# coganlab/cross_patient_speech_decoding

Hardware: AMD Instinct MI355X
Metric: ECoG trials/sec seq2seq-RNN training (higher is better)
Workload: dtype bf16x3; 1 GPU; configs[3] per-GPU shard: 8-patient MCCA-aligned input (d = 30), enc 2x bi-GRU H=512, dec 1x GRU, T=200 (T'=20), F=100, full-batch step of 2048 trials per GPU (8 patients x 2048 trials over 8 GPUs), dropout 0.3, teacher forcing 0.5, clip 0.5, AdamW; trials_per_gpu=2048, global_batch=2048, parallelism=dp1, collective=none (single process)

## Files before the change

### cross_patient_speech_decoding_amd/csrc/xps_gemm.hip

```cpp
#include <stdlib.h>
#include <string.h>
#include <atomic>
#include "xps_common.h"
#include "xps_gemm_tile.h"
#include "xps_gemm_big.h"
#include "xps_gemm_dma.h"
using namespace xps_tile;
#ifndef XPS_GEMM_DEFAULT_MODE
#define XPS_GEMM_DEFAULT_MODE 1
#endif
namespace {

#ifndef XPS_BF_MI1_WAVES
#define XPS_BF_MI1_WAVES XPS_GEMM_WAVES
#endif
template <bool AK, bool BK, int MI, bool EDGE = false, bool BF = false, bool PRE = false>
__global__ __launch_bounds__(256, (BF && MI == 1) ? XPS_BF_MI1_WAVES : XPS_GEMM_WAVES) void gemm_f32_kernel(
    const float* __restrict__ A, RowMap ra, const float* __restrict__ B, RowMap rb,
    const float* __restrict__ A2, const float* __restrict__ B2, int K2,
    float* __restrict__ C, RowMap rc, const float* __restrict__ bias,
    int M, int N, int K, int kchunk, long long slab_stride, int accumulate, int vecA, int vecB) {
    __shared__ __attribute__((aligned(16))) TileMem<BF, MI> mem;
    const int tiles_n = (N + BN - 1) / BN, tiles = tiles_n * ((M + 64 * MI - 1) / (64 * MI));
    const int lid = xcd_remap(blockIdx.x, gridDim.x);
    const int z = lid / tiles, t = lid % tiles;
    const int kbeg = z * kchunk;
    const int kend = min(K, kbeg + kchunk);
    const int m0 = (t / tiles_n) * (64 * MI), n0 = (t % tiles_n) * BN;
    f32x16 acc[MI][2];
    zero_acc<MI>(acc);
    float nocs = 0.f;
    f32x4 nocs4 = {0.f, 0.f, 0.f, 0.f};
    gemm_accumulate_any<AK, BK, MI, EDGE, BF, PRE>(acc, nocs, nocs4, false, A, ra, B, rb, M, N, K, m0, n0, kbeg, kend, vecA, vecB, mem);
    if (A2) gemm_accumulate_any<AK, BK, MI, EDGE, BF, PRE>(acc, nocs, nocs4, false, A2, ra, B2, rb, M, N, K2, m0, n0, 0, K2, vecA, vecB, mem);
    gemm_store<MI>(acc, C + (long long)z * slab_stride, rc, bias, M, N, m0, n0, accumulate);
}

constexpr int SM_MAXM = 16, SM_SLICES = 16, SM_KC = 1024;
template <bool AK, bool BK>
__global__ __launch_bounds__(1024) void gemm_small_kernel(
    const float* __restrict__ A, RowMap ra, const float* __restrict__ B, RowMap rb,
    const float* __restrict__ A2, const float* __restrict__ B2, int K2,
    float* __restrict__ C, RowMap rc, const float* __restrict__ bias, int M, int N, int K, int accumulate, int vecB) {
    __shared__ __attribute__((aligned(16))) float As[SM_MAXM][SM_KC];
    __shared__ float red[SM_SLICES][SM_MAXM][64];
    const int tid = threadIdx.x, l = tid & 63, w = tid >> 6;
    const int n = blockIdx.x * 64 + l;
    float acc[SM_MAXM];
#pragma unroll
    for (int m = 0; m < SM_MAXM; ++m) acc[m] = 0.f;
    for (int pass = 0; pass < 2; ++pass) {
        const float* __restrict__ Ap = pass ? A2 : A;
// ... 27 lines not shown
                    }
#pragma unroll
                    for (int m = 0; m < SM_MAXM; ++m) {
                        const f32x4 a = *reinterpret_cast<const f32x4*>(&As[m][k]);
                        acc[m] += a.x * b[0]; acc[m] += a.y * b[1]; acc[m] += a.z * b[2]; acc[m] += a.w * b[3];
                    }
                }
                for (; k < k1; ++k) {
                    const float b = BK ? Bp[boff + k] : Bp[(plain_b ? (long long)(kc + k) * rb.ld : rb.off(kc + k)) + boff];
#pragma unroll
                    for (int m = 0; m < SM_MAXM; ++m) acc[m] += As[m][k] * b;
                }
            }
        }
    }
#pragma unroll
    for (int m = 0; m < SM_MAXM; ++m) red[w][m][l] = acc[m];
    __syncthreads();
    if (w < M && n < N) {
        float v = 0.f;
#pragma unroll
        for (int s = 0; s < SM_SLICES; ++s) v += red[s][w][l];
        if (bias) v += bias[n];
        float* c = C + rc.off(w) + n;
        if (accumulate) v += *c;
        *c = v;
    }
}

struct NtMulti {
    const float* B[4];
    const float* bias[4];
    float* C[4];
};
template <int MI, bool EDGE = false, bool BF = false, bool PRE = false>
__global__ __launch_bounds__(256, (BF && MI == 1) ? XPS_BF_MI1_WAVES : XPS_GEMM_WAVES) void gemm_nt_multi_kernel(
    const float* __restrict__ A, RowMap ra, NtMulti pm, RowMap rb, RowMap rc, int M, int N, int K, int nprob,
    int vecA, int vecB) {
    __shared__ __attribute__((aligned(16))) TileMem<BF, MI> mem;
    const int tiles_n = (N + BN - 1) / BN;
    const int lid = xcd_remap(blockIdx.x, gridDim.x);
    const int per_m = nprob * tiles_n, rem = lid % per_m;
    const int z = rem / tiles_n;
    const int m0 = (lid / per_m) * (64 * MI), n0 = (rem % tiles_n) * BN;
    f32x16 acc[MI][2];
    zero_acc<MI>(acc);
    float nocs = 0.f;
    f32x4 nocs4 = {0.f, 0.f, 0.f, 0.f};
    gemm_accumulate_any<true, true, MI, EDGE, BF, PRE>(acc, nocs, nocs4, false, A, ra, pm.B[z], rb, M, N, K, m0, n0, 0, K, vecA, vecB, mem);
    gemm_store<MI>(acc, pm.C[z], rc, pm.bias[z], M, N, m0, n0, 0);
}


template <int KT>
__global__ __launch_bounds__(512, 1) void proj_ws_kernel(const float* __restrict__ A, long long lda, NtMulti pm, long long ldb, long long ldc,
                                                         int M, int N, int K, int nprob, int preA, int preB) {
    constexpr int KP = 16 * KT;
#ifndef XPS_WS_PAD
#define XPS_WS_PAD 4
#endif
    constexpr int LDH = ((KP / 2 + 63) / 64) * 64 + XPS_WS_PAD;
    constexpr int NV = KP / 32;
    extern __shared__ __attribute__((aligned(16))) unsigned char ws_smem[];
    unsigned* lds = reinterpret_cast<unsigned*>(ws_smem);
    const int tid = threadIdx.x, lane = tid & 63, wave = tid >> 6;
    const int NC = nprob * N, S = (NC + 255) / 256;
    const int lid = xcd_remap(blockIdx.x, gridDim.x);
    const int slice = lid % S, rg = lid / S;
    const int nb = (gridDim.x - slice + S - 1) / S;
    const int c0 = slice * 256 + wave * 32;
    const bool active = c0 < NC;
    const int z = active ? c0 / N : 0, n0 = active ? c0 % N : 0;
    const int li = lane & 31, lk = lane >> 5;

    bf16x8 wh[KT], wl[KT];
    {
        const float* wrow = pm.B[z] + (long long)(n0 + li) * ldb;
#pragma unroll
        for (int kk = 0; kk < KT; ++kk) {
            const int k = 16 * kk + 8 * lk;
            f32x4 v0 = {0.f, 0.f, 0.f, 0.f}, v1 = v0;
            if (active && k < K) v0 = *reinterpret_cast<const f32x4*>(wrow + k);
            if (active && k + 4 < K) v1 = *reinterpret_cast<const f32x4*>(wrow + k + 4);
            bf16x4 h0, l0, h1, l1;
            stage_split(v0, preB != 0, h0, l0);
            stage_split(v1, preB != 0, h1, l1);
            wh[kk] = __builtin_shufflevector(h0, h1, 0, 1, 2, 3, 4, 5, 6, 7);
            wl[kk] = __builtin_shufflevector(l0, l1, 0, 1, 2, 3, 4, 5, 6, 7);
        }
    }
    float bv = 0.f;
    if (active && pm.bias[z]) bv = pm.bias[z][n0 + li];

    const int tiles = (M + 63) / 64;
    auto load_tile = [&](int t, f32x4 (&r)[NV]) {
#pragma unroll
        for (int j = 0; j < NV; ++j) {
            const int v = tid + 512 * j, row = t * 64 + v / (KP / 4), k = 4 * (v % (KP / 4));
            r[j] = (row < M && k < K) ? *reinterpret_cast<const f32x4*>(A + (long long)row * lda + k) : f32x4{0.f, 0.f, 0.f, 0.f};
        }
    };
    auto store_tile = [&](const f32x4 (&r)[NV], int buf) {
        unsigned* hi = lds + (size_t)buf * 2 * 64 * LDH;
        unsigned* lo = hi + 64 * LDH;
#pragma unroll
        for (int j = 0; j < NV; ++j) {
            const int v = tid + 512 * j, row = v / (KP / 4), kd = 2 * (v % (KP / 4));
            bf16x4 h, l;
            stage_split(r[j], preA != 0, h, l);
            *reinterpret_cast<bf16x4*>(hi + row * LDH + kd) = h;
            *reinterpret_cast<bf16x4*>(lo + row * LDH + kd) = l;
        }
    };

    f32x4 raw[NV];
    int t = rg;
    if (t < tiles) load_tile(t, raw);
    for (int it = 0; t < tiles; t += nb, ++it) {
        const int buf = it & 1;
        store_tile(raw, buf);
        if (t + nb < tiles) load_tile(t + nb, raw);
        __syncthreads();
        if (active) {
            const unsigned* hi = lds + (size_t)buf * 2 * 64 * LDH;
            const unsigned* lo = hi + 64 * LDH;
            f32x16 acc[2];
#pragma unroll
            for (int i = 0; i < 2; ++i)
#pragma unroll
                for (int r = 0; r < 16; ++r) acc[i][r] = 0.f;
#pragma unroll
            for (int kk = 0; kk < KT; ++kk) {
#pragma unroll
                for (int i = 0; i < 2; ++i) {
                    const int off = (32 * i + li) * LDH + 8 * kk + 4 * lk;
                    const bf16x8 ah = *reinterpret_cast<const bf16x8*>(hi + off);
                    const bf16x8 al = *reinterpret_cast<const bf16x8*>(lo + off);
                    acc[i] = __builtin_amdgcn_mfma_f32_32x32x16_bf16(al, wh[kk], acc[i], 0, 0, 0);
                    acc[i] = __builtin_amdgcn_mfma_f32_32x32x16_bf16(ah, wl[kk], acc[i], 0, 0, 0);
                    acc[i] = __builtin_amdgcn_mfma_f32_32x32x16_bf16(ah, wh[kk], acc[i], 0, 0, 0);
                }
            }
            float* cbase = pm.C[z] + n0 + li;
#pragma unroll
            for (int i = 0; i < 2; ++i)
#pragma unroll
                for (int r = 0; r < 16; ++r) {
                    const int row = t * 64 + 32 * i + (r & 3) + 8 * (r >> 2) + 4 * lk;
                    if (row < M) __builtin_nontemporal_store(acc[i][r] + bv, cbase + (long long)row * ldc);
                }
        }
    }
}
constexpr int proj_ws_lds(int KT) { return 2 * 2 * 64 * (((16 * KT / 2 + 63) / 64) * 64 + XPS_WS_PAD) * 4; }

constexpr int TN_MAXP = 12;
struct TnProb {
    const float* A; const float* B; float* C; float* colsum;
    RowMap ra, rb, rc;
    int M, N, K, accumulate;
    int splits, kchunk, tiles_n, vecA, vecB;
    long long slab_off;
    int block_start;
    int big;
};
struct TnGroup {
    TnProb p[TN_MAXP];
    int n;
    int total_blocks;
    int total_blocks_big;
    long long total_out;
    int uniform, tiles_all;
    int tile_start[TN_MAXP];
};

constexpr int TN_TILE = BM * BN;
__host__ __device__ inline long long tn_split_stride(long long ntiles, int M, bool has_colsum) {
    return ntiles * TN_TILE + (has_colsum ? ((M + 3) & ~3) : 0);
}
__device__ inline void slab_store(const f32x16 (&acc)[2][2], float* __restrict__ tile) {
    const int lane = threadIdx.x & 63, wave = threadIdx.x >> 6;
    float* base = tile + wave * 4096 + lane * 4;
#pragma unroll
    for (int i = 0; i < 2; ++i)
#pragma unroll
        for (int j = 0; j < 2; ++j)
#pragma unroll
            for (int q = 0; q < 4; ++q) {
                const f32x4 v = {acc[i][j][4 * q], acc[i][j][4 * q + 1], acc[i][j][4 * q + 2], acc[i][j][4 * q + 3]};
                __builtin_nontemporal_store(v, reinterpret_cast<f32x4*>(base + ((i * 2 + j) * 4 + q) * 256));
            }
}
__device__ inline void slab_decode(int e, int& row, int& col) {
    const int wave = e >> 12, ij = (e >> 10) & 3, q = (e >> 8) & 3, lane = (e >> 2) & 63, c = e & 3;
    const int reg = 4 * q + c, li = lane & 31, lk = lane >> 5;
    row = (wave >> 1) * 64 + (ij >> 1) * 32 + (reg & 3) + 8 * (reg >> 2) + 4 * lk;
    col = (wave & 1) * 64 + (ij & 1) * 32 + li;
}

template <bool EDGE, bool BF = false, bool PRE = false>
__global__ __launch_bounds__(256, XPS_GEMM_WAVES) void gemm_tn_grouped_kernel(TnGroup g, float* __restrict__ ws) {
    __shared__ __attribute__((aligned(16))) TileMem<BF> mem;
    const int lid = xcd_remap(blockIdx.x, gridDim.x);
    int pi = 0, local;
    if (g.uniform) {
        const int zz = lid / g.tiles_all, rem = lid - zz * g.tiles_all;
#pragma unroll 1
// ... 179 lines not shown
    }
}

extern __shared__ __attribute__((aligned(16))) unsigned char big_smem[];

template <bool AK, bool BK, bool DEEP, int FMT = -1>
__device__ inline void big_accumulate(f32x16 (&acc)[4][2], f32x4& csum, bool want_csum, const float* __restrict__ A, long long lda,
                                      const float* __restrict__ B, long long ldb, int m0, int n0, int kbeg, int kend,
                                      const bool preA = false, const bool preB = false) {
    if constexpr (DEEP) {
        xps_big::BigStage32& st = *reinterpret_cast<xps_big::BigStage32*>(big_smem);
        xps_big::BigLoader32<AK> la;
        xps_big::BigLoader32<BK> lb;
        la.init(A, lda, m0, kbeg, threadIdx.x);
        lb.init(B, ldb, n0, kbeg, threadIdx.x);
        xps_big::big_pipeline32<AK, BK>(acc, csum, want_csum, la, lb, (kend - kbeg) / 32, st, preA, preB);
    } else {
        xps_big::BigStage& st = *reinterpret_cast<xps_big::BigStage*>(big_smem);
        xps_big::BigLoader<AK> la;
        xps_big::BigLoader<BK> lb;
        la.init(A, lda, m0, kbeg, threadIdx.x);
        lb.init(B, ldb, n0, kbeg, threadIdx.x);
        if constexpr (FMT >= 0) xps_big::big_pipeline_t<AK, BK, (FMT & 1) != 0, (FMT & 2) != 0>(acc, csum, want_csum, la, lb, (kend - kbeg) / BKT, st);
        else xps_big::big_pipeline<AK, BK>(acc, csum, want_csum, la, lb, (kend - kbeg) / BKT, st, preA, preB);
    }
}

template <bool AK, bool BK, bool DEEP, int FMT = 0>
__global__ __launch_bounds__(512, 1) void gemm_big_kernel(const float* __restrict__ A, long long lda, const float* __restrict__ B,
                                                           long long ldb, const float* __restrict__ A2, const float* __restrict__ B2,
                                                           int K2, float* __restrict__ C, long long ldc,
                                                           const float* __restrict__ bias, int N, int K, int accumulate, int fmt) {
    const int tiles_n = FMT == 5 ? 1 : N / xps_big::TN;
    const int lid = xcd_remap(blockIdx.x, gridDim.x);
    const int m0 = (lid / tiles_n) * xps_big::TM, n0 = (lid % tiles_n) * xps_big::TN;
    f32x16 acc[4][2];
    xps_big::big_zero(acc);
    f32x4 nocs = {0.f, 0.f, 0.f, 0.f};
    if constexpr (FMT == 5) {
        const bool act = (int)((threadIdx.x >> 6) & 3) * 64 < N;
        xps_big::direct_dma_pipeline<!BK>(acc, A, lda, B, ldb, m0, 0, 0, K / 32, big_smem, act);
        if (A2) xps_big::direct_dma_pipeline<!BK>(acc, A2, lda, B2, ldb, m0, 0, 0, K2 / 32, big_smem, act);
        xps_big::big_store_c_masked(acc, C, ldc, bias, m0, N, accumulate);
        return;
    }
    if constexpr (FMT == 4) {
        xps_big::direct_dma_pipeline<!BK>(acc, A, lda, B, ldb, m0, n0, 0, K / 32, big_smem);
        if (A2) xps_big::direct_dma_pipeline<!BK>(acc, A2, lda, B2, ldb, m0, n0, 0, K2 / 32, big_smem);
    } else {
        big_accumulate<AK, BK, DEEP, DEEP ? -1 : FMT>(acc, nocs, false, A, lda, B, ldb, m0, n0, 0, K, !DEEP && (fmt & 1) != 0, !DEEP && (fmt & 2) != 0);
        if (A2) big_accumulate<AK, BK, DEEP, DEEP ? -1 : FMT>(acc, nocs, false, A2, lda, B2, ldb, m0, n0, 0, K2, !DEEP && (fmt & 1) != 0, !DEEP && (fmt & 2) != 0);
    }
    xps_big::big_store_c(acc, C, ldc, bias, m0, n0, accumulate);
}

template <bool DEEP, bool DMA = false>
__global__ __launch_bounds__(512, 1) void gemm_big_nt_multi_kernel(const float* __restrict__ A, long long lda, NtMulti pm, long long ldb,
                                                                    long long ldc, int N, int K, int nprob, int fmt) {
    const int tiles_n = N / xps_big::TN;
    const int lid = xcd_remap(blockIdx.x, gridDim.x);
    const int per_m = nprob * tiles_n, rem = lid % per_m;
    const int z = rem / tiles_n;
    const int m0 = (lid / per_m) * xps_big::TM, n0 = (rem % tiles_n) * xps_big::TN;
    f32x16 acc[4][2];
    xps_big::big_zero(acc);
    f32x4 nocs = {0.f, 0.f, 0.f, 0.f};
    if constexpr (DMA) xps_big::direct_dma_pipeline<false>(acc, A, lda, pm.B[z], ldb, m0, n0, 0, K / 32, big_smem);
    else big_accumulate<true, true, DEEP>(acc, nocs, false, A, lda, pm.B[z], ldb, m0, n0, 0, K, !DEEP && (fmt & 1) != 0, !DEEP && (fmt & 2) != 0);
    xps_big::big_store_c(acc, pm.C[z], ldc, pm.bias[z], m0, n0, 0);
}

template <bool DEEP>
__global__ __launch_bounds__(512, 1) void gemm_big_tn_kernel(TnGroup g, float* __restrict__ ws) {
    const int lid = xcd_remap(blockIdx.x, gridDim.x);
    int pi = -1;
#pragma unroll 1
    for (int i = 0; i < g.n; ++i)
        if (g.p[i].big && lid >= g.p[i].block_start) pi = i;
    const TnProb& P = g.p[pi];
    const int local = lid - P.block_start;
    const int tiles_n = P.N / xps_big::TN, ntiles = (P.M / xps_big::TM) * tiles_n;
    const int tile = local % ntiles, z = local / ntiles;
    const int tm = tile / tiles_n, tn = tile % tiles_n;
    const int kbeg = z * P.kchunk, kend = min(P.K, kbeg + P.kchunk);
    const long long ntiles128 = (long long)(P.M / BM) * P.tiles_n;
    const long long split_stride = tn_split_stride(ntiles128, P.M, P.colsum != nullptr);
    float* slab = ws + P.slab_off + (long long)z * split_stride;
    const bool want_cs = P.colsum && tn == 0;
    f32x16 acc[4][2];
    xps_big::big_zero(acc);
    if (!DEEP && P.big == 2) {
        f32x16 cacc;
#pragma unroll
        for (int r = 0; r < 16; ++r) cacc[r] = 0.f;
        const int per = (8 + tiles_n - 1) / tiles_n;
        const int cs_lo = min(8, tn * per), cs_hi = min(8, cs_lo + per);
        const bool cs_here = P.colsum && cs_lo < cs_hi;
        if (cs_here) xps_big::tn_dma_pipeline<true>(acc, cacc, P.A, P.ra.ld, P.B, P.rb.ld, tm * xps_big::TM, tn * xps_big::TN, kbeg, (kend - kbeg) / BKT, big_smem, cs_lo, cs_hi);
        else xps_big::tn_dma_pipeline<false>(acc, cacc, P.A, P.ra.ld, P.B, P.rb.ld, tm * xps_big::TM, tn * xps_big::TN, kbeg, (kend - kbeg) / BKT, big_smem);
        float* subd[4];
#pragma unroll
        for (int s = 0; s < 4; ++s)
            subd[s] = slab + ((long long)(2 * tm + (s >> 1)) * P.tiles_n + 2 * tn + (s & 1)) * TN_TILE;
        xps_big::big_slab_store(acc, subd);
        if (cs_here) xps_big::dma_colsum_store(cacc, slab + ntiles128 * TN_TILE + tm * xps_big::TM, cs_lo, cs_hi);
        return;
// ... 39 lines not shown
inline bool aligned16(const void* p) { return (reinterpret_cast<uintptr_t>(p) & 15) == 0; }
inline bool map_vec_ok(const float* p, const RowMap& r) {
    return aligned16(p) && (r.ld % 4 == 0) && (r.gs % 4 == 0);
}
inline int split4_flag(const float* p, const RowMap& r, long long extent) {
    if (r.fmt == 0) return 0;
    if (r.fmt != 1 || !map_vec_ok(p, r) || extent % 4 != 0) return -1;
    return 2;
}

int tn_splits(int M, int N, int K) {
    long long tiles = (long long)cdiv(M, BM) * cdiv(N, BN);
    int want = (int)((768 + tiles - 1) / tiles);
    int maxs = cdiv(K, 256);
    int s = want < maxs ? want : maxs;
    if (s < 1) s = 1;
    if (s > 256) s = 256;
    return s;
}

}

namespace {
std::atomic<int>& gemm_mode() {
    static std::atomic<int> mode([] {
        const char* e = getenv("XPS_GEMM_PRECISION");
        if (e && (!strcmp(e, "fp32") || !strcmp(e, "f32") || !strcmp(e, "0"))) return 0;
        if (e && (!strcmp(e, "bf16x3") || !strcmp(e, "1"))) return 1;
        return XPS_GEMM_DEFAULT_MODE;
    }());
    return mode;
}
inline bool bf_mode() { return gemm_mode().load(std::memory_order_relaxed) == 1; }

inline bool use_small_tiles(int M, int N, int K = 0) {
    static const int thr = [] {
        const char* e = getenv("XPS_GEMM_SMALL_TILE_BLOCKS");
        int v = e ? atoi(e) : -1;
        return v >= 0 ? v : 2048;
    }();
    const long long n128 = (long long)cdiv(M, 128) * cdiv(N, BN);
    static const bool longk = [] { const char* e = getenv("XPS_GEMM_LONGK_128"); return !(e && e[0] == '0'); }();
    if (longk && K >= 1024 && n128 >= 512) return false;
    return M > 64 && n128 < thr;
}

std::atomic<int>& big_switch() {
    static std::atomic<int> on([] { const char* e = getenv("XPS_GEMM_BIG"); return (e && e[0] == '0') ? 0 : 1; }());
    return on;
}
inline bool big_enabled() { return big_switch().load(std::memory_order_relaxed) != 0 && bf_mode(); }
inline bool dma_enabled() { const char* e = getenv("XPS_GEMM_DMA"); return !(e && e[0] == '0'); }
inline bool proj_ws_enabled() { const char* e = getenv("XPS_PROJ_WS"); return !(e && e[0] == '0'); }
inline bool big_plain(const float* p, const RowMap& r, int rows) { return aligned16(p) && r.ld % 4 == 0 && r.rpg >= rows; }
constexpr int BIG_LDS = (int)sizeof(xps_big::BigStage), BIG_LDS32 = (int)sizeof(xps_big::BigStage32);
constexpr int BIG_TN_LDS = BIG_LDS > xps_big::DMA_LDS ? BIG_LDS : xps_big::DMA_LDS;
template <typename Kern>
inline bool big_prepare(Kern kern, int bytes) {
    return hipFuncSetAttribute(reinterpret_cast<const void*>(kern), hipFuncAttributeMaxDynamicSharedMemorySize, bytes) == hipSuccess;
}
inline bool big_deep_allowed() {
    static const bool on = [] { const char* e = getenv("XPS_GEMM_BIG_DEEP"); return e && e[0] == '1'; }();
    return on;
}
inline int big_min_tiles() {
    static const int v = [] { const char* e = getenv("XPS_GEMM_BIG_MIN_TILES"); int x = e ? atoi(e) : 0; return x > 0 ? x : 192; }();
    return v;
}

inline int device_cus() {
    static const int cus = [] {
        int dev = 0, n = 0;
        if (hipGetDevice(&dev) == hipSuccess && hipDeviceGetAttribute(&n, hipDeviceAttributeMultiprocessorCount, dev) == hipSuccess && n > 0) return n;
        return 256;
    }();
    return cus;
}
inline int big_split_rows(int M, int tiles_per_row_tile) {
    static const bool on = [] { const char* e = getenv("XPS_GEMM_BIG_TAIL"); return !(e && e[0] == '0'); }();
    const int cus = device_cus();
    const long long mt = M / xps_big::TM, total = mt * tiles_per_row_tile;
    const long long rounds = total / cus, rem = total % cus;
    if (!on || rounds < 1 || rem == 0 || rem * 4 > (long long)cus * 3) return M;
    const long long mb = (rounds * cus) / tiles_per_row_tile;
    if (mb < 1 || mb >= mt) return M;
    return (int)(mb * xps_big::TM);
}

template <bool AK, bool BK>
int launch_gemm(const float* A, const RowMap& ra, const float* B, const RowMap& rb, const float* A2, const float* B2, int K2,
                float* C, const RowMap& rc, const float* bias, int M, int N, int K, int accumulate, hipStream_t st) {
    const int kchunk = ((K + BKT - 1) / BKT) * BKT + BKT;
    int vecA = (int)(map_vec_ok(A, ra) && (!A2 || map_vec_ok(A2, ra)));
    int vecB = (int)(map_vec_ok(B, rb) && (!B2 || map_vec_ok(B2, rb)));
    int fA = split4_flag(A, ra, AK ? K : M), fB = split4_flag(B, rb, BK ? K : N);
    if (A2 && fA > 0) fA = split4_flag(A2, ra, AK ? K2 : M);
    if (B2 && fB > 0) fB = split4_flag(B2, rb, BK ? K2 : N);
    if (fA < 0 || fB < 0 || ((fA | fB) && (!bf_mode() || M <= SM_MAXM))) return -2;
    vecA |= fA; vecB |= fB;
    const int fmt = (fA ? 1 : 0) | (fB ? 2 : 0);
    if (M <= SM_MAXM) {
        hipLaunchKernelGGL((gemm_small_kernel<AK, BK>), dim3(cdiv(N, 64)), dim3(1024), 0, st, A, ra, B, rb, A2, B2, K2, C, rc,
                           bias, M, N, K, accumulate, vecB);
        return hipGetLastError() == hipSuccess ? 0 : -1;
    }
    if constexpr (AK && !BK) {
        if (big_enabled() && dma_enabled() && fmt == 3 && N < xps_big::TN && N % 4 == 0 && rb.ld >= xps_big::TN && M % xps_big::TM == 0 &&
            M / xps_big::TM >= 96 && K % 32 == 0 && K2 % 32 == 0 && K + K2 >= 512 && big_plain(A, ra, M) && big_plain(B, rb, K) &&
            (!A2 || (big_plain(A2, ra, M) && big_plain(B2, rb, K2))) && rc.rpg >= M) {
            constexpr int lds = xps_big::direct_dma_lds<true>();
            static const bool ready5 = big_prepare(gemm_big_kernel<true, false, false, 5>, lds);
            if (ready5) {
                hipLaunchKernelGGL((gemm_big_kernel<true, false, false, 5>), dim3(M / xps_big::TM), dim3(xps_big::NTHR), lds, st,
                                   A, ra.ld, B, rb.ld, A2, B2, K2, C, rc.ld, bias, N, K, accumulate, fmt);
                return hipGetLastError() == hipSuccess ? 0 : -1;
            }
        }
    }
    if (big_enabled() && M % xps_big::TM == 0 && N % xps_big::TN == 0 && K % BKT == 0 && K2 % BKT == 0 && K >= 64 &&
        (long long)(M / xps_big::TM) * (N / xps_big::TN) >= big_min_tiles() &&
        big_plain(A, ra, AK ? M : K) && big_plain(B, rb, BK ? N : K) && (!A2 || (big_plain(A2, ra, AK ? M : K2) && big_plain(B2, rb, BK ? N : K2))) &&
        rc.rpg >= M) {
        static const bool ready = big_prepare(gemm_big_kernel<AK, BK, false, 0>, BIG_LDS) && big_prepare(gemm_big_kernel<AK, BK, false, 1>, BIG_LDS) &&
                                  big_prepare(gemm_big_kernel<AK, BK, false, 2>, BIG_LDS) && big_prepare(gemm_big_kernel<AK, BK, false, 3>, BIG_LDS) &&
                                  big_prepare(gemm_big_kernel<AK, BK, true>, BIG_LDS32);
        if (ready) {
            const int Mfull = M;
            M = big_split_rows(M, N / xps_big::TN);
            const dim3 bgrid((M / xps_big::TM) * (N / xps_big::TN));
            const int Mtail = Mfull - M;
            auto run_tail = [&]() -> int {
                if (Mtail <= 0) return 0;
                const float* At = AK ? A + (long long)M * ra.ld : A + M;
                const float* A2t = A2 ? (AK ? A2 + (long long)M * ra.ld : A2 + M) : nullptr;
                return launch_gemm<AK, BK>(At, ra, B, rb, A2t, B2, K2, C + (long long)M * rc.ld, rc, bias, Mtail, N, K, accumulate, st);
            };
            bool dma_done = false;
            if constexpr (AK) {
                if (fmt == 3 && K % 32 == 0 && K2 % 32 == 0 && dma_enabled()) {
                    constexpr int lds = xps_big::direct_dma_lds<!BK>();
                    static const bool ready4 = big_prepare(gemm_big_kernel<AK, BK, false, 4>, lds);
                    if (ready4) {
                        hipLaunchKernelGGL((gemm_big_kernel<AK, BK, false, 4>), bgrid, dim3(xps_big::NTHR), lds, st,
                                           A, ra.ld, B, rb.ld, A2, B2, K2, C, rc.ld, bias, N, K, accumulate, fmt);
                        dma_done = true;
                    }
                }
            }
            if (dma_done) {
            } else if (big_deep_allowed() && K % 32 == 0 && K2 % 32 == 0 && fmt == 0)
                hipLaunchKernelGGL((gemm_big_kernel<AK, BK, true>), bgrid, dim3(xps_big::NTHR), BIG_LDS32, st,
                                   A, ra.ld, B, rb.ld, A2, B2, K2, C, rc.ld, bias, N, K, accumulate, fmt);
            else if (fmt == 0)
                hipLaunchKernelGGL((gemm_big_kernel<AK, BK, false, 0>), bgrid, dim3(xps_big::NTHR), BIG_LDS, st,
                                   A, ra.ld, B, rb.ld, A2, B2, K2, C, rc.ld, bias, N, K, accumulate, fmt);
            else if (fmt == 1)
                hipLaunchKernelGGL((gemm_big_kernel<AK, BK, false, 1>), bgrid, dim3(xps_big::NTHR), BIG_LDS, st,
                                   A, ra.ld, B, rb.ld, A2, B2, K2, C, rc.ld, bias, N, K, accumulate, fmt);
            else if (fmt == 2)
// ... 57 lines not shown
    XPS_CHECK_ARG(A && B && C && ra_ && rb_ && rc_, "null argument");
    XPS_CHECK_ARG(M >= 0 && N >= 0 && K >= 0, "negative size");
    if (M == 0 || N == 0) return XPS_OK;
    RowMap ra = to_rowmap(ra_), rb = to_rowmap(rb_), rc = to_rowmap(rc_);
    const int lrc = launch_gemm<true, false>(A, ra, B, rb, nullptr, nullptr, 0, C, rc, nullptr, M, N, K, accumulate, (hipStream_t)stream);
    if (lrc == -2) {
        xps_set_error("xps_gemm_nn_f32: XPS_FMT_SPLIT4 operand needs bf16x3 mode, M > 16, 16-byte aligned rows and a contiguous extent that is a multiple of 4");
        return XPS_E_INVALID;
    }
    if (lrc) {
        xps_set_error("xps_gemm_nn_f32: launch failed: %s", hipGetErrorString(hipGetLastError()));
        return XPS_E_HIP;
    }
    return XPS_OK;
}

extern "C" int xps_gemm_nt_multi_f32(const float* A, const xps_rowmap* ra_, const float* const* B, const xps_rowmap* rb_,
                                     float* const* C, const xps_rowmap* rc_, const float* const* bias, int nprob,
                                     int M, int N, int K, void* stream) {
    XPS_CHECK_ARG(A && B && C && ra_ && rb_ && rc_, "null argument");
    XPS_CHECK_ARG(nprob >= 1 && nprob <= 4, "1..4 problems");
    XPS_CHECK_ARG(M >= 0 && N >= 0 && K >= 0, "negative size");
    if (M == 0 || N == 0) return XPS_OK;
    RowMap ra = to_rowmap(ra_), rb = to_rowmap(rb_), rc = to_rowmap(rc_);
    NtMulti pm;
    bool vb = true;
    for (int i = 0; i < 4; ++i) {
        const int j = i < nprob ? i : 0;
        XPS_CHECK_ARG(B[j] && C[j], "null problem pointer");
        pm.B[i] = B[j]; pm.C[i] = C[j]; pm.bias[i] = bias ? bias[j] : nullptr;
        vb = vb && map_vec_ok(B[j], rb);
    }
    int vecA = (int)map_vec_ok(A, ra), vecB = (int)vb;
    int fA = split4_flag(A, ra, K), fB = 0;
    for (int i = 0; i < nprob && fB >= 0; ++i) fB = split4_flag(B[i], rb, K);
    if (fA < 0 || fB < 0 || ((fA | fB) && !bf_mode())) {
        xps_set_error("xps_gemm_nt_multi_f32: XPS_FMT_SPLIT4 operand needs bf16x3 mode, 16-byte aligned rows and K %% 4 == 0");
        return XPS_E_INVALID;
    }
    vecA |= fA; vecB |= fB;
    const int fmt = (fA ? 1 : 0) | (fB ? 2 : 0);
    if (bf_mode() && proj_ws_enabled() && K >= 32 && K <= 256 && K % 4 == 0 && N % 32 == 0 && (long long)nprob * N >= 256 && M >= 4096 &&
        vecA && vb && ra.rpg >= M && rb.rpg >= N && rc.rpg >= M) {
        const int KT = 2 * ((K + 31) / 32);
        static const int cus = [] {
            int dev = 0, n = 0;
            if (hipGetDevice(&dev) == hipSuccess && hipDeviceGetAttribute(&n, hipDeviceAttributeMultiprocessorCount, dev) == hipSuccess && n > 0) return n;
            return 256;
        }();
        const int S = cdiv((long long)nprob * N, 256), tiles = cdiv(M, 64);
        int grid = cus < tiles * S ? cus : tiles * S;
        grid = (grid / S) * S;
        if (grid >= S) {
#define XPS_LAUNCH_WS(KT_)                                                                                                            \
    do {                                                                                                                              \
        static const bool ok_ = big_prepare(proj_ws_kernel<KT_>, proj_ws_lds(KT_));                                                    \
        if (!ok_) { xps_set_error("xps_gemm_nt_multi_f32: cannot reserve %d bytes of LDS", proj_ws_lds(KT_)); return XPS_E_HIP; }       \
        hipLaunchKernelGGL(proj_ws_kernel<KT_>, dim3(grid), dim3(512), proj_ws_lds(KT_), (hipStream_t)stream, A, ra.ld, pm, rb.ld, rc.ld, \
                           M, N, K, nprob, fA ? 1 : 0, fB ? 1 : 0);                                                                      \
    } while (0)
            switch (KT) {
                case 2: XPS_LAUNCH_WS(2); break;
                case 4: XPS_LAUNCH_WS(4); break;
                case 6: XPS_LAUNCH_WS(6); break;
                case 8: XPS_LAUNCH_WS(8); break;
                case 10: XPS_LAUNCH_WS(10); break;
                case 12: XPS_LAUNCH_WS(12); break;
                case 14: XPS_LAUNCH_WS(14); break;
                default: XPS_LAUNCH_WS(16); break;
            }
#undef XPS_LAUNCH_WS
            XPS_CHECK_LAUNCH();
            return XPS_OK;
        }
    }
    if (big_enabled() && M % xps_big::TM == 0 && N % xps_big::TN == 0 && K % BKT == 0 && K >= 64 && vb &&
        (long long)(M / xps_big::TM) * (N / xps_big::TN) * nprob >= big_min_tiles() &&
        big_plain(A, ra, M) && rb.rpg >= N && rc.rpg >= M) {
        static const bool ready = big_prepare(gemm_big_nt_multi_kernel<false>, BIG_LDS) && big_prepare(gemm_big_nt_multi_kernel<true>, BIG_LDS32);
        if (ready) {
            const int Mfull = M;
            M = big_split_rows(M, (N / xps_big::TN) * nprob);
            const dim3 bgrid((M / xps_big::TM) * (N / xps_big::TN) * nprob);
            static const bool ready_dma = big_prepare(gemm_big_nt_multi_kernel<false, true>, xps_big::direct_dma_lds<false>());
            if (fmt == 3 && K % 32 == 0 && dma_enabled() && ready_dma)
                hipLaunchKernelGGL((gemm_big_nt_multi_kernel<false, true>), bgrid, dim3(xps_big::NTHR), xps_big::direct_dma_lds<false>(),
                                   (hipStream_t)stream, A, ra.ld, pm, rb.ld, rc.ld, N, K, nprob, fmt);
            else if (big_deep_allowed() && K % 32 == 0 && fmt == 0)
                hipLaunchKernelGGL(gemm_big_nt_multi_kernel<true>, bgrid, dim3(xps_big::NTHR), BIG_LDS32, (hipStream_t)stream, A, ra.ld, pm,
                                   rb.ld, rc.ld, N, K, nprob, fmt);
            else
                hipLaunchKernelGGL(gemm_big_nt_multi_kernel<false>, bgrid, dim3(xps_big::NTHR), BIG_LDS,
                               (hipStream_t)stream, A, ra.ld, pm, rb.ld, rc.ld, N, K, nprob, fmt);
            XPS_CHECK_LAUNCH();
            if (Mfull > M) {
                float* Ct[4];
                for (int i = 0; i < nprob; ++i) Ct[i] = C[i] + (long long)M * rc.ld;
                return xps_gemm_nt_multi_f32(A + (long long)M * ra.ld, ra_, B, rb_, Ct, rc_, bias, nprob, Mfull - M, N, K, stream);
            }
            return XPS_OK;
        }
    }
#define XPS_LAUNCH_NTM(MI_, EDGE_, BF_)                                                                                  \
    do {                                                                                                                 \
        if (BF_ && fmt)                                                                                                  \
            hipLaunchKernelGGL((gemm_nt_multi_kernel<MI_, EDGE_, BF_, BF_>), dim3(cdiv(N, BN) * cdiv(M, 64 * MI_) * nprob), dim3(256), 0, \
                               (hipStream_t)stream, A, ra, pm, rb, rc, M, N, K, nprob, vecA, vecB);                        \
        else                                                                                                             \
            hipLaunchKernelGGL((gemm_nt_multi_kernel<MI_, EDGE_, BF_>), dim3(cdiv(N, BN) * cdiv(M, 64 * MI_) * nprob), dim3(256), 0,    \
                               (hipStream_t)stream, A, ra, pm, rb, rc, M, N, K, nprob, vecA, vecB);                        \
    } while (0)
    const bool bf = bf_mode();
// ... 278 lines not shown
```

### cross_patient_speech_decoding_amd/csrc/xps_gemm_dma.h

```cpp
#pragma once
#include <type_traits>
#include "xps_gemm_big.h"

namespace xps_big {

#ifndef XPS_DMA_STAGES
#define XPS_DMA_STAGES 4
#endif
constexpr int DMA_D = XPS_DMA_STAGES;
constexpr int DMA_ROW = 1024;
constexpr int DMA_QPAD = 144;
constexpr int DMA_IMG = 16 * DMA_ROW + 4 * DMA_QPAD;
constexpr int DMA_STAGE = 2 * DMA_IMG;
constexpr int DMA_LDS = DMA_D * DMA_STAGE;
#ifndef XPS_DMA_SHIFT8
#define XPS_DMA_SHIFT8 1
#endif
__host__ __device__ constexpr int dma_rowoff(int k) {
    return k * DMA_ROW + (k >> 2) * DMA_QPAD + ((k & 1) ? (XPS_DMA_SHIFT8 ? 8 : 0) : 0) + ((k & 2) ? 128 : 0);
}
constexpr int DMA_ROW4 = 4 * DMA_ROW + DMA_QPAD;

#ifdef XPS_DMA_STAMP
__device__ unsigned long long g_dma_stamp[4096 * 4];
// ... 375 lines not shown
    unsigned long long u0 = 0, u1 = 0, u2 = 0, u3 = 0, u4 = 0, u5 = 0, z_wait = 0, z_bar = 0, z_mma = 0, z_bar2 = 0, z_dma = 0;
#endif
    for (int ks = 0; ks < nks; ++ks) {
        DSTAMP(u0)
        asm volatile("s_waitcnt vmcnt(8)" ::: "memory");
        DSTAMP(u1)
        __builtin_amdgcn_s_barrier();
        DSTAMP(u2)
        const unsigned char* sa = smem + (ks & 1) * STAGE;
        const unsigned char* sb = sa + KC_IMG;
        if (active)
#pragma unroll
        for (int t = 0; t < 2; ++t) {
            bf16x8 bh[2], bl[2];
#pragma unroll
            for (int j = 0; j < 2; ++j) {
                if (BKX) frag_kx(sb, wn + 32 * j, t, bh[j], bl[j]);
                else frag_kc(sb, wn + 32 * j, t, bh[j], bl[j]);
            }
#pragma unroll
            for (int i = 0; i < 4; ++i) {
                bf16x8 ah, al;
                frag_kc(sa, wm + 32 * i, t, ah, al);
#pragma unroll
                for (int j = 0; j < 2; ++j) {
                    acc[i][j] = __builtin_amdgcn_mfma_f32_32x32x16_bf16(al, bh[j], acc[i][j], 0, 0, 0);
                    acc[i][j] = __builtin_amdgcn_mfma_f32_32x32x16_bf16(ah, bl[j], acc[i][j], 0, 0, 0);
                    acc[i][j] = __builtin_amdgcn_mfma_f32_32x32x16_bf16(ah, bh[j], acc[i][j], 0, 0, 0);
                }
            }
        }
        asm volatile("s_waitcnt lgkmcnt(0)" ::: "memory");
        DSTAMP(u3)
        __builtin_amdgcn_s_barrier();
        DSTAMP(u4)
#pragma unroll
        for (int pc = 0; pc < 8; ++pc) piece(ks + 2, pc);
#ifdef XPS_DMA_STAMP
        DSTAMP(u5)
        z_wait += u1 - u0; z_bar += u2 - u1; z_mma += u3 - u2; z_bar2 += u4 - u3; z_dma += u5 - u4;
#endif
    }
#ifdef XPS_DMA_STAMP
    if (lane == 0) {
        unsigned long long* o = g_dma_stamp + ((blockIdx.x * 8 + wave) & 4095) * 4;
        o[0] = z_wait; o[1] = z_bar + z_bar2; o[2] = z_dma; o[3] = z_mma;
    }
#endif
#endif
    asm volatile("s_waitcnt vmcnt(0)" ::: "memory");
    __builtin_amdgcn_s_barrier();
}

}
```

Before: 312,300 trials/s.

## Add skinny NN GEMM DMA kernel and LDS-bounced wide stores for projection

Result: faster. 316,200 trials/s, median of 6 (+1.2%).

```diff
diff --git a/cross_patient_speech_decoding_amd/csrc/xps_gemm.hip b/cross_patient_speech_decoding_amd/csrc/xps_gemm.hip
--- a/cross_patient_speech_decoding_amd/csrc/xps_gemm.hip
+++ b/cross_patient_speech_decoding_amd/csrc/xps_gemm.hip
@@ -1,3 +1,4 @@
+#include <stdint.h>
 #include <stdlib.h>
 #include <string.h>
 #include <atomic>
@@ -131,13 +132,22 @@
 }
 
 
-template <int KT>
-__global__ __launch_bounds__(512, 1) void proj_ws_kernel(const float* __restrict__ A, long long lda, NtMulti pm, long long ldb, long long ldc,
-                                                         int M, int N, int K, int nprob, int preA, int preB) {
-    constexpr int KP = 16 * KT;
 #ifndef XPS_WS_PAD
 #define XPS_WS_PAD 4
 #endif
+constexpr int proj_ws_lds(int KT) { return 2 * 2 * 64 * (((16 * KT / 2 + 63) / 64) * 64 + XPS_WS_PAD) * 4; }
+constexpr int WS_BLD = 36;
+constexpr int proj_ws_bounce_rows(int KT) { return KT <= 8 ? 32 : 16; }
+constexpr int proj_ws_lds_wide(int KT) { return proj_ws_lds(KT) + 8 * proj_ws_bounce_rows(KT) * WS_BLD * 4; }
+__device__ inline void wave_lds_sync() {
+    __builtin_amdgcn_fence(__ATOMIC_RELEASE, "wavefront");
+    __builtin_amdgcn_wave_barrier();
+    __builtin_amdgcn_fence(__ATOMIC_ACQUIRE, "wavefront");
+}
+template <int KT>
+__global__ __launch_bounds__(512, 1) void proj_ws_kernel(const float* __restrict__ A, long long lda, NtMulti pm, long long ldb, long long ldc,
+                                                         int M, int N, int K, int nprob, int preA, int preB, int wide) {
+    constexpr int KP = 16 * KT;
     constexpr int LDH = ((KP / 2 + 63) / 64) * 64 + XPS_WS_PAD;
     constexpr int NV = KP / 32;
     extern __shared__ __attribute__((aligned(16))) unsigned char ws_smem[];
@@ -220,18 +230,42 @@
                     acc[i] = __builtin_amdgcn_mfma_f32_32x32x16_bf16(ah, wh[kk], acc[i], 0, 0, 0);
                 }
             }
-            float* cbase = pm.C[z] + n0 + li;
-#pragma unroll
-            for (int i = 0; i < 2; ++i)
-#pragma unroll
-                for (int r = 0; r < 16; ++r) {
-                    const int row = t * 64 + 32 * i + (r & 3) + 8 * (r >> 2) + 4 * lk;
-                    if (row < M) __builtin_nontemporal_store(acc[i][r] + bv, cbase + (long long)row * ldc);
-                }
-        }
-    }
-}
-constexpr int proj_ws_lds(int KT) { return 2 * 2 * 64 * (((16 * KT / 2 + 63) / 64) * 64 + XPS_WS_PAD) * 4; }
+            if (wide) {
+                constexpr int BR = proj_ws_bounce_rows(KT), RP = BR / 2;
+                float* bt = reinterpret_cast<float*>(ws_smem + proj_ws_lds(KT)) + wave * (BR * WS_BLD);
+                float* cw = pm.C[z] + n0 + 4 * (lane & 7);
+#pragma unroll
+                for (int i = 0; i < 2; ++i)
+#pragma unroll
+                    for (int p = 0; p < 32 / BR; ++p) {
+#pragma unroll
+                        for (int q = 0; q < RP; ++q) {
+                            const int r = RP * p + q;
+                            bt[((q & 3) + 8 * (q >> 2) + 4 * lk) * WS_BLD + li] = acc[i][r] + bv;
+                        }
+                        wave_lds_sync();
+#pragma unroll
+                        for (int j = 0; j < BR / 8; ++j) {
+                            const int lr = 8 * j + (lane >> 3);
+                            const f32x4 v = *reinterpret_cast<const f32x4*>(bt + lr * WS_BLD + 4 * (lane & 7));
+                            const int row = t * 64 + 32 * i + BR * p + lr;
+                            if (row < M) __builtin_nontemporal_store(v, reinterpret_cast<f32x4*>(cw + (long long)row * ldc));
+                        }
+                        wave_lds_sync();
+                    }
+            } else {
+                float* cbase = pm.C[z] + n0 + li;
+#pragma unroll
+                for (int i = 0; i < 2; ++i)
+#pragma unroll
+                    for (int r = 0; r < 16; ++r) {
+                        const int row = t * 64 + 32 * i + (r & 3) + 8 * (r >> 2) + 4 * lk;
+                        if (row < M) __builtin_nontemporal_store(acc[i][r] + bv, cbase + (long long)row * ldc);
+                    }
+            }
+        }
+    }
+}
 
 constexpr int TN_MAXP = 12;
 struct TnProb {
@@ -517,6 +551,34 @@
         if (A2) big_accumulate<AK, BK, DEEP, DEEP ? -1 : FMT>(acc, nocs, false, A2, lda, B2, ldb, m0, n0, 0, K2, !DEEP && (fmt & 1) != 0, !DEEP && (fmt & 2) != 0);
     }
     xps_big::big_store_c(acc, C, ldc, bias, m0, n0, accumulate);
+}
+
+__global__ __launch_bounds__(256, 1) void gemm_skinny_nn_kernel(const float* __restrict__ A, const float* __restrict__ B, int K,
+                                                                const float* __restrict__ A2, const float* __restrict__ B2, int K2,
+                                                                long long lda, long long ldb, float* __restrict__ C, long long ldc,
+                                                                int M, int N, int accumulate) {
+    const int m0 = blockIdx.x * xps_big::SK_TM;
+    f32x16 acc[xps_big::SK_TM / 32];
+#pragma unroll
+    for (int i = 0; i < xps_big::SK_TM / 32; ++i)
+#pragma unroll
+        for (int r = 0; r < 16; ++r) acc[i][r] = 0.f;
+    xps_big::skinny_nn_pipeline(acc, A, B, K / 32, A2, B2, A2 ? K2 / 32 : 0, lda, ldb, m0, M, N, big_smem);
+    const int lane = threadIdx.x & 63, wave = threadIdx.x >> 6;
+    const int n = 32 * wave + (lane & 31), lk = lane >> 5;
+    if (n >= N) return;
+#pragma unroll
+    for (int i = 0; i < xps_big::SK_TM / 32; ++i)
+#pragma unroll
+        for (int r = 0; r < 16; ++r) {
+            const int row = m0 + 32 * i + (r & 3) + 8 * (r >> 2) + 4 * lk;
+            if (row < M) {
+                float* c = C + (long long)row * ldc + n;
+                float v = acc[i][r] + 0.f;
+                if (accumulate) v += *c;
+                __builtin_nontemporal_store(v, c);
+            }
+        }
 }
 
 template <bool DEEP, bool DMA = false>
@@ -662,6 +724,17 @@
 inline bool big_enabled() { return big_switch().load(std::memory_order_relaxed) != 0 && bf_mode(); }
 inline bool dma_enabled() { const char* e = getenv("XPS_GEMM_DMA"); return !(e && e[0] == '0'); }
 inline bool proj_ws_enabled() { const char* e = getenv("XPS_PROJ_WS"); return !(e && e[0] == '0'); }
+inline bool proj_ws_wide_enabled() { const char* e = getenv("XPS_PROJ_WS_WIDE"); return !(e && e[0] == '0'); }
+inline bool proj_ws_wide_ok(bool enabled, bool c_aligned128, long long ldc, int N) { return enabled && c_aligned128 && ldc % 32 == 0 && N % 32 == 0; }
+inline int skinny_nn_mode() { const char* e = getenv("XPS_SKINNY_NN"); return !e ? 1 : (e[0] == '0' ? 0 : (e[0] == '2' ? 2 : 1)); }
+inline bool skinny_nn_shape_ok(int M, int N, int K, int K2) {
+    return M > 0 && N >= 4 && N <= 128 && N % 4 == 0 && K >= 32 && K % 32 == 0 && K2 >= 0 && K2 % 32 == 0;
+}
+inline bool skinny_nn_wanted(int mode, int cus, int M, int N, int K, int K2) {
+    if (mode == 0 || !skinny_nn_shape_ok(M, N, K, K2)) return false;
+    if (mode == 2) return true;
+    return (long long)M * 4 >= (long long)cus * xps_big::SK_TM && K + K2 >= 512;
+}
 inline bool big_plain(const float* p, const RowMap& r, int rows) { return aligned16(p) && r.ld % 4 == 0 && r.rpg >= rows; }
 constexpr int BIG_LDS = (int)sizeof(xps_big::BigStage), BIG_LDS32 = (int)sizeof(xps_big::BigStage32);
 constexpr int BIG_TN_LDS = BIG_LDS > xps_big::DMA_LDS ? BIG_LDS : xps_big::DMA_LDS;
@@ -715,6 +788,16 @@
         return hipGetLastError() == hipSuccess ? 0 : -1;
     }
     if constexpr (AK && !BK) {
+        if (bf_mode() && fmt == 1 && !bias && skinny_nn_wanted(skinny_nn_mode(), device_cus(), M, N, K, A2 ? K2 : 0) &&
+            big_plain(A, ra, M) && (!A2 || big_plain(A2, ra, M)) && aligned16(B) && (!B2 || aligned16(B2)) && rb.ld % 4 == 0 && rb.ld >= N &&
+            rb.rpg >= (K > K2 ? K : K2) && rc.rpg >= M && ra.ld * 4 * xps_big::SK_TM < (1LL << 32) && rb.ld * 4 * 8 < (1LL << 32)) {
+            static const bool ready_sk = big_prepare(gemm_skinny_nn_kernel, xps_big::SK_LDS);
+            if (ready_sk) {
+                hipLaunchKernelGGL(gemm_skinny_nn_kernel, dim3(cdiv(M, xps_big::SK_TM)), dim3(256), xps_big::SK_LDS, st,
+                                   A, B, K, A2, B2, K2, ra.ld, rb.ld, C, rc.ld, M, N, accumulate);
+                return hipGetLastError() == hipSuccess ? 0 : -1;
+            }
+        }
         if (big_enabled() && dma_enabled() && fmt == 3 && N < xps_big::TN && N % 4 == 0 && rb.ld >= xps_big::TN && M % xps_big::TM == 0 &&
             M / xps_big::TM >= 96 && K % 32 == 0 && K2 % 32 == 0 && K + K2 >= 512 && big_plain(A, ra, M) && big_plain(B, rb, K) &&
             (!A2 || (big_plain(A2, ra, M) && big_plain(B2, rb, K2))) && rc.rpg >= M) {
@@ -878,12 +961,15 @@
         int grid = cus < tiles * S ? cus : tiles * S;
         grid = (grid / S) * S;
         if (grid >= S) {
+            bool c128 = true;
+            for (int i = 0; i < nprob; ++i) c128 = c128 && (reinterpret_cast<uintptr_t>(C[i]) % 128 == 0);
+            const int wide = (int)proj_ws_wide_ok(proj_ws_wide_enabled(), c128, rc.ld, N);
 #define XPS_LAUNCH_WS(KT_)                                                                                                            \
     do {                                                                                                                              \
-        static const bool ok_ = big_prepare(proj_ws_kernel<KT_>, proj_ws_lds(KT_));                                                    \
-        if (!ok_) { xps_set_error("xps_gemm_nt_multi_f32: cannot reserve %d bytes of LDS", proj_ws_lds(KT_)); return XPS_E_HIP; }       \
-        hipLaunchKernelGGL(proj_ws_kernel<KT_>, dim3(grid), dim3(512), proj_ws_lds(KT_), (hipStream_t)stream, A, ra.ld, pm, rb.ld, rc.ld, \
-                           M, N, K, nprob, fA ? 1 : 0, fB ? 1 : 0);                                                                      \
+        static const bool ok_ = big_prepare(proj_ws_kernel<KT_>, proj_ws_lds_wide(KT_));                                               \
+        if (!ok_) { xps_set_error("xps_gemm_nt_multi_f32: cannot reserve %d bytes of LDS", proj_ws_lds_wide(KT_)); return XPS_E_HIP; }  \
+        hipLaunchKernelGGL(proj_ws_kernel<KT_>, dim3(grid), dim3(512), wide ? proj_ws_lds_wide(KT_) : proj_ws_lds(KT_),                 \
+                           (hipStream_t)stream, A, ra.ld, pm, rb.ld, rc.ld, M, N, K, nprob, fA ? 1 : 0, fB ? 1 : 0, wide);               \
     } while (0)
             switch (KT) {
                 case 2: XPS_LAUNCH_WS(2); break;
diff --git a/cross_patient_speech_decoding_amd/csrc/xps_gemm_dma.h b/cross_patient_speech_decoding_amd/csrc/xps_gemm_dma.h
--- a/cross_patient_speech_decoding_amd/csrc/xps_gemm_dma.h
+++ b/cross_patient_speech_decoding_amd/csrc/xps_gemm_dma.h
@@ -451,4 +451,94 @@
     __builtin_amdgcn_s_barrier();
 }
 
-}
+constexpr int SK_TM = 160, SK_D = 4;
+constexpr int SK_A_STAGE = SK_TM * 128;
+constexpr int SK_B_STAGE = 32 * 512 + 4 * 128;
+constexpr int SK_LDS = SK_D * (SK_A_STAGE + SK_B_STAGE);
+__host__ __device__ constexpr int sk_brow(int k) { return k * 512 + (k >> 3) * 128; }
+
+__device__ inline void skinny_nn_pipeline(f32x16 (&acc)[SK_TM / 32], const float* __restrict__ A1, const float* __restrict__ B1, int n1,
+                                          const float* __restrict__ A2, const float* __restrict__ B2, int n2, long long lda,
+                                          long long ldb, int m0, int M, int N, unsigned char* smem) {
+    const int tid = threadIdx.x, lane = tid & 63;
+    const int wave = __builtin_amdgcn_readfirstlane(tid >> 6);
+    const unsigned lds0 = dma_lds_base(smem);
+    const int ns = n1 + n2;
+    if (ns <= 0) return;
+    const int rr = lane >> 3, cpos = lane & 7;
+    const int keyw = ((8 * wave + rr) >> 1) & 7;
+    unsigned va[5];
+#pragma unroll
+    for (int j = 0; j < 5; ++j) {
+        int row = 8 * (wave + 4 * j) + rr;
+        row = row < M - m0 ? row : M - m0 - 1;
+        va[j] = (unsigned)((long long)row * lda * 4 + ((cpos ^ keyw) * 16));
+    }
+    const int bg = lane & 31;
+    const unsigned vb = (unsigned)((long long)(2 * wave + (lane >> 5)) * ldb * 4 + (bg * 4 < N ? bg * 16 : 0));
+    const long long bstep = 8 * ldb * 4;
+    const unsigned char* a1 = reinterpret_cast<const unsigned char*>(A1 + (long long)m0 * lda);
+    const unsigned char* a2 = reinterpret_cast<const unsigned char*>(A2 ? A2 + (long long)m0 * lda : A1 + (long long)m0 * lda);
+    const unsigned char* b1 = reinterpret_cast<const unsigned char*>(B1);
+    const unsigned char* b2 = reinterpret_cast<const unsigned char*>(B2 ? B2 : B1);
+    auto pieces = [&](int s) {
+        const int ss = s < ns ? s : ns - 1;
+        const bool second = ss >= n1;
+        const int kk = second ? ss - n1 : ss;
+        const unsigned char* ab = (second ? a2 : a1) + (long long)kk * 128;
+        const unsigned char* bb = (second ? b2 : b1) + (long long)kk * 32 * ldb * 4;
+        const unsigned sa = lds0 + (unsigned)(s % SK_D) * SK_A_STAGE;
+        const unsigned sb = lds0 + SK_D * SK_A_STAGE + (unsigned)(s % SK_D) * SK_B_STAGE;
+#pragma unroll
+        for (int j = 0; j < 5; ++j) dma_piece(ab, va[j], sa + (unsigned)(wave + 4 * j) * 1024u);
+#pragma unroll
+        for (int j = 0; j < 4; ++j) dma_piece(bb + j * bstep, vb, sb + (unsigned)sk_brow(2 * (wave + 4 * j)));
+    };
+    const int r = lane & 31, h = lane >> 5, key = (r >> 1) & 7;
+    int fka[2][2];
+#pragma unroll
+    for (int t = 0; t < 2; ++t)
+#pragma unroll
+        for (int j = 0; j < 2; ++j) fka[t][j] = r * 128 + (((4 * t + 2 * h + j) ^ key) << 4);
+    const int n = 32 * wave + r;
+    const bool n_ok = n < N, active = 32 * wave < N;
+    const int fb = h * (8 * 512 + 128) + n * 4;
+#pragma unroll
+    for (int d = 0; d < SK_D - 1; ++d) pieces(d);
+    for (int s = 0; s < ns; ++s) {
+        asm volatile("s_waitcnt vmcnt(18)" ::: "memory");
+        __builtin_amdgcn_s_barrier();
+        pieces(s + SK_D - 1);
+        if (active) {
+            const unsigned char* sa = smem + (s % SK_D) * SK_A_STAGE;
+            const unsigned char* sb = smem + SK_D * SK_A_STAGE + (s % SK_D) * SK_B_STAGE + fb;
+#pragma unroll
+            for (int t = 0; t < 2; ++t) {
+                bf16x8 bh, bl;
+#pragma unroll
+                for (int j = 0; j < 8; ++j) {
+                    float v = *reinterpret_cast<const float*>(sb + (16 * t + j) * 512 + t * 256);
+                    if (!n_ok) v = 0.f;
+                    __bf16 x, y;
+                    xps_tile::bf_split(v, x, y);
+                    bh[j] = x; bl[j] = y;
+                }
+#pragma unroll
+                for (int i = 0; i < SK_TM / 32; ++i) {
+                    const bf16x8 ga = *reinterpret_cast<const bf16x8*>(sa + i * 32 * 128 + fka[t][0]);
+                    const bf16x8 gb = *reinterpret_cast<const bf16x8*>(sa + i * 32 * 128 + fka[t][1]);
+                    const bf16x8 ah = __builtin_shufflevector(ga, gb, 0, 1, 2, 3, 8, 9, 10, 11);
+                    const bf16x8 al = __builtin_shufflevector(ga, gb, 4, 5, 6, 7, 12, 13, 14, 15);
+                    acc[i] = __builtin_amdgcn_mfma_f32_32x32x16_bf16(al, bh, acc[i], 0, 0, 0);
+                    acc[i] = __builtin_amdgcn_mfma_f32_32x32x16_bf16(ah, bl, acc[i], 0, 0, 0);
+                    acc[i] = __builtin_amdgcn_mfma_f32_32x32x16_bf16(ah, bh, acc[i], 0, 0, 0);
+                }
+            }
+        }
+        asm volatile("s_waitcnt lgkmcnt(0)" ::: "memory");
+    }
+    asm volatile("s_waitcnt vmcnt(0)" ::: "memory");
+    __builtin_amdgcn_s_barrier();
+}
+
+}
```
